# microsoft/MoGe

Measured on AMD Instinct MI355X. Metric: images/sec (MoGeModel.infer, moge-2-vitl 518x518 fp16), higher is better.
Workload: dtype f16

## Files before the change

moge_amd/csrc/attention_pp.hip:

```cpp
#include "common.h"

#define AP_GPTR(p) ((const __attribute__((address_space(1))) void*)(p))
#define AP_LPTR(p) ((__attribute__((address_space(3))) void*)(p))

typedef short s16x4 __attribute__((ext_vector_type(4)));

__device__ __forceinline__ u32x4 tr_pair(const char* p0, const char* p1) {
    const s16x4 a = __builtin_amdgcn_ds_read_tr16_b64_v4i16((__attribute__((address_space(3))) s16x4*)(p0));
    const s16x4 b = __builtin_amdgcn_ds_read_tr16_b64_v4i16((__attribute__((address_space(3))) s16x4*)(p1));
    typedef short s16x8 __attribute__((ext_vector_type(8)));
    const s16x8 v = {a[0], a[1], a[2], a[3], b[0], b[1], b[2], b[3]};
    return __builtin_bit_cast(u32x4, v);
}

__device__ __forceinline__ u32x4 pack8(const f32x16& p, int s) {
    f16x8 h;
#pragma unroll
    for (int i = 0; i < 8; i++) h[i] = (f16)p[8 * s + i];
    return __builtin_bit_cast(u32x4, h);
}

constexpr int AP_STAGE = 16384;
constexpr float AP_PSUM_LIMIT = 16384.f;

#ifdef MOGE_EXPERIMENTS
#include "../../tools/experiments/attention_pp_exp.inc"
#endif

constexpr int AP_VAR_DEFAULT = 0;
constexpr int AP_X_DEFAULT = 0;
constexpr int AP_KERN_DEFAULT = 3;
constexpr float AP_SCORE_LIMIT = 15.f;
constexpr float AP_ROWSUM_LIMIT = 49152.f;
template <int VAR>
__global__ __launch_bounds__(256, 3) void attn_pp16_kernel(const f16* __restrict__ q, const f16* __restrict__ k, const f16* __restrict__ v,
                                                           f16* __restrict__ out, int Ntok, int nh) {
    constexpr int NW = 4, NPW = 4;
    extern __shared__ __attribute__((aligned(16))) char smem[];

    const int tid = threadIdx.x, lane = tid & 63;
    const int wave = __builtin_amdgcn_readfirstlane(tid >> 6);
    const int l15 = lane & 15, g4 = lane >> 4;
    const int bh = blockIdx.y;
    const int b = bh / nh, head = bh - b * nh;
    const int q0 = blockIdx.x * (NW * 32) + wave * 32;

    u32x4 qf[2][2];
#pragma unroll
    for (int qb = 0; qb < 2; qb++) {
        const int qrow = q0 + qb * 16 + l15;
        const f16* qp = q + ((size_t)bh * Ntok + (qrow < Ntok ? qrow : Ntok - 1)) * 64;
#pragma unroll
        for (int ks = 0; ks < 2; ks++) qf[qb][ks] = *reinterpret_cast<const u32x4*>(qp + 32 * ks + 8 * g4);
    }

    const char* kbase = reinterpret_cast<const char*>(k + (size_t)bh * Ntok * 64);
    const char* vbase = reinterpret_cast<const char*>(v + (size_t)bh * Ntok * 64);
    const int prow = lane >> 3, pch = lane & 7;
    int drow[NPW];
    unsigned doff[NPW];
#pragma unroll
    for (int i = 0; i < NPW; i++) {
        const int p = wave + NW * i;
        const int row = (p & 7) * 8 + prow;
        drow[i] = row;
        const int ksw = ((row >> 1) & 1) | (((row >> 3) & 3) << 1);
        const int vsw = (((row >> 1) & 1) << 1) | (((row >> 3) & 1) << 2);
        doff[i] = (unsigned)(row * 128 + ((pch ^ (p >= 8 ? vsw : ksw)) << 4));
    }
    const int ntiles = (Ntok + 63) >> 6;
    auto issue = [&](int t) {
        char* st = smem + (t % 3) * AP_STAGE;
        const char* kt = uniform_ptr(kbase + (size_t)t * 8192);
        const char* vt = uniform_ptr(vbase + (size_t)t * 8192);
        if (t < ntiles - 1) {
#pragma unroll
            for (int i = 0; i < NPW; i++) {
                const int p = wave + NW * i;
                __builtin_amdgcn_global_load_lds(AP_GPTR((p >= 8 ? vt : kt) + doff[i]), AP_LPTR(st + p * 1024), 16, 0, 0);
            }
        } else {
#pragma unroll
            for (int i = 0; i < NPW; i++) {
                const int p = wave + NW * i;
                const int over = t * 64 + drow[i] - (Ntok - 1);
                const unsigned off = doff[i] - (over > 0 ? (unsigned)over * 128u : 0u);
                __builtin_amdgcn_global_load_lds(AP_GPTR((p >= 8 ? vt : kt) + off), AP_LPTR(st + p * 1024), 16, 0, 0);
            }
        }
    };

    const int kswl = ((l15 >> 1) & 1) | ((l15 >> 2) << 1);
    int kaddr[2];
#pragma unroll
    for (int ks = 0; ks < 2; ks++) kaddr[ks] = (8 * (l15 >> 2) + (l15 & 3)) * 128 + (((4 * ks + g4) ^ kswl) << 4);
    const int vswl = (((l15 >> 3) & 1) << 1) | ((g4 & 1) << 2);
    int vaddr[4];
#pragma unroll
    for (int db = 0; db < 4; db++)
        vaddr[db] = 8192 + (8 * g4 + (l15 >> 2)) * 128 + ((((2 * db) ^ vswl) | ((l15 & 3) >> 1)) << 4) + (l15 & 1) * 8;

    f32x4 o[4][2];
    f32x4 negs[2];
    float m_run[2], l_run[2];
#pragma unroll
    for (int qb = 0; qb < 2; qb++) {
#pragma unroll
        for (int db = 0; db < 4; db++) o[db][qb] = f32x4{0.f, 0.f, 0.f, 0.f};
        negs[qb] = f32x4{0.f, 0.f, 0.f, 0.f};
        m_run[qb] = -1e30f; l_run[qb] = 0.f;
    }

    issue(0);
    if (ntiles > 1) issue(1);

    int stage = 0;
    const char* ka[2];
    const char* va[4];
    f32x4 sc[4][2];
    float psum[2];
    auto tile_head = [&](int t) {
        if (t + 1 < ntiles) asm volatile("s_waitcnt vmcnt(%0)" ::"n"(NPW) : "memory");
        else asm volatile("s_waitcnt vmcnt(0)" ::: "memory");
        __builtin_amdgcn_s_barrier();
        asm volatile("" ::: "memory");
        if (t + 2 < ntiles) issue(t + 2);
        const int so = stage * AP_STAGE;
        stage = stage == 2 ? 0 : stage + 1;
#pragma unroll
        for (int ks = 0; ks < 2; ks++) ka[ks] = smem + (kaddr[ks] + so);
#pragma unroll
        for (int db = 0; db < 4; db++) va[db] = smem + (vaddr[db] + so);
    };
    auto pv = [&]() {
#pragma unroll
        for (int qb = 0; qb < 2; qb++) l_run[qb] += psum[qb];
#pragma unroll
        for (int s2 = 0; s2 < 2; s2++) {
            u32x4 pf[2];
#pragma unroll
            for (int qb = 0; qb < 2; qb++) {
                f16x8 hp;
#pragma unroll
                for (int r = 0; r < 4; r++) { hp[r] = (f16)sc[2 * s2][qb][r]; hp[4 + r] = (f16)sc[2 * s2 + 1][qb][r]; }
                pf[qb] = __builtin_bit_cast(u32x4, hp);
            }
#pragma unroll
            for (int db = 0; db < 4; db++) {
                const u32x4 vf = tr_pair(va[db] + (32 * ((VAR & 32) ? 0 : s2)) * 128, va[db] + (32 * ((VAR & 32) ? 0 : s2) + 4) * 128);
#pragma unroll
                for (int qb = 0; qb < 2; qb++) mma16<f16>(o[db][qb], vf, pf[qb]);
            }
        }
    };
    auto exact_body = [&](int t, bool last) {
#pragma unroll
        for (int kb = 0; kb < 4; kb++) {
            const int koff = (32 * (kb >> 1) + 4 * (kb & 1)) * 128;
            const u32x4 kf0 = *reinterpret_cast<const u32x4*>(ka[0] + koff), kf1 = *reinterpret_cast<const u32x4*>(ka[1] + koff);
#pragma unroll
            for (int qb = 0; qb < 2; qb++) {
                sc[kb][qb] = f32x4{0.f, 0.f, 0.f, 0.f};
                mma16<f16>(sc[kb][qb], kf0, qf[qb][0]);
                mma16<f16>(sc[kb][qb], kf1, qf[qb][1]);
            }
        }
#pragma unroll
        for (int qb = 0; qb < 2; qb++) {
            if (last) {
#pragma unroll
                for (int kb = 0; kb < 4; kb++)
#pragma unroll
                    for (int r = 0; r < 4; r++) {
                        const int key = t * 64 + 32 * (kb >> 1) + 8 * g4 + 4 * (kb & 1) + r;
                        if (key >= Ntok) sc[kb][qb][r] = -1e30f;
                    }
            }
            float mx = sc[0][qb][0];
#pragma unroll
            for (int kb = 0; kb < 4; kb++)
#pragma unroll
                for (int r = 0; r < 4; r++) mx = fmaxf(mx, sc[kb][qb][r]);
            mx = fmaxf(mx, __shfl_xor(mx, 16));
            mx = fmaxf(mx, __shfl_xor(mx, 32));
            const float m_new = fmaxf(m_run[qb], mx);
            const float alpha = __builtin_amdgcn_exp2f(m_run[qb] - m_new);
            m_run[qb] = m_new;
            l_run[qb] *= alpha;
#pragma unroll
            for (int db = 0; db < 4; db++)
#pragma unroll
                for (int r = 0; r < 4; r++) o[db][qb][r] *= alpha;
#pragma unroll
            for (int r = 0; r < 4; r++) negs[qb][r] = -m_new;
            float ps = 0.f;
#pragma unroll
            for (int kb = 0; kb < 4; kb++)
#pragma unroll
                for (int r = 0; r < 4; r++) {
                    sc[kb][qb][r] = __builtin_amdgcn_exp2f(sc[kb][qb][r] - m_new);
                    ps += sc[kb][qb][r];
                }
            psum[qb] = ps;
        }
        pv();
    };

    tile_head(0);
    exact_body(0, ntiles == 1);
    int t = 1;
    for (;;) {
        bool hit = false;
        for (; t < ntiles - 1; t++) {
            tile_head(t);
            if constexpr (VAR & 4) {
                u32x4 kf[4][2];
#pragma unroll
                for (int kb = 0; kb < 4; kb++) {
                    const int koff = (32 * (kb >> 1) + 4 * (kb & 1)) * 128;
                    kf[kb][0] = *reinterpret_cast<const u32x4*>(ka[0] + koff);
                    kf[kb][1] = *reinterpret_cast<const u32x4*>(ka[1] + koff);
                }
#pragma unroll
                for (int kb = 0; kb < 4; kb++)
#pragma unroll
                    for (int qb = 0; qb < 2; qb++)
                        sc[kb][qb] = __builtin_amdgcn_mfma_f32_16x16x32_f16(__builtin_bit_cast(f16x8, kf[kb][0]), __builtin_bit_cast(f16x8, qf[qb][0]), negs[qb], 0, 0, 0);
#pragma unroll
                for (int kb = 0; kb < 4; kb++)
#pragma unroll
                    for (int qb = 0; qb < 2; qb++) mma16<f16>(sc[kb][qb], kf[kb][1], qf[qb][1]);
            } else {
#pragma unroll
            for (int kb = 0; kb < 4; kb++) {
                const int koff = (32 * (kb >> 1) + 4 * (kb & 1)) * 128;
                const u32x4 kf0 = *reinterpret_cast<const u32x4*>(ka[0] + koff), kf1 = *reinterpret_cast<const u32x4*>(ka[1] + koff);
#pragma unroll
                for (int qb = 0; qb < 2; qb++) {
                    sc[kb][qb] = __builtin_amdgcn_mfma_f32_16x16x32_f16(__builtin_bit_cast(f16x8, kf0), __builtin_bit_cast(f16x8, qf[qb][0]), negs[qb], 0, 0, 0);
                    mma16<f16>(sc[kb][qb], kf1, qf[qb][1]);
                }
            }
            }
            bool trig = false;
            if constexpr ((VAR & 8) != 0) {
                float mx = sc[0][0][0];
#pragma unroll
                for (int kb = 0; kb < 4; kb++)
#pragma unroll
                    for (int qb = 0; qb < 2; qb++)
#pragma unroll
                        for (int r = 0; r < 4; r++) mx = fmaxf(mx, sc[kb][qb][r]);
                trig = !(mx <= AP_SCORE_LIMIT);
                if (__builtin_expect(__any(trig), 0)) { hit = true; break; }
            }
#pragma unroll
            for (int qb = 0; qb < 2; qb++) {
                float ps0 = 0.f, ps1 = 0.f;
#pragma unroll
                for (int kb = 0; kb < 4; kb++)
#pragma unroll
                    for (int r = 0; r < 4; r++) {
                        sc[kb][qb][r] = (VAR & 1) ? sc[kb][qb][r] * 1e-3f : __builtin_amdgcn_exp2f(sc[kb][qb][r]);
                        if (!(VAR & 16) || (kb == 0 && r == 0)) { if (kb & 1) ps1 += sc[kb][qb][r]; else ps0 += sc[kb][qb][r]; }
                    }
                psum[qb] = ps0 + ps1;
                trig |= !(psum[qb] < AP_PSUM_LIMIT);
            }
            if constexpr ((VAR & (2 | 8)) == 0) {
                if (__builtin_expect(__any(trig), 0)) { hit = true; break; }
            }
            pv();
        }
        if (!hit) break;
        exact_body(t, false);
        t++;
    }
    if (ntiles > 1) {
        tile_head(ntiles - 1);
        exact_body(ntiles - 1, true);
    }
#pragma unroll
    for (int qb = 0; qb < 2; qb++) {
        float l_tot = l_run[qb] + __shfl_xor(l_run[qb], 16);
        l_tot += __shfl_xor(l_tot, 32);
        const float inv = 1.f / l_tot;
        const int qrow = q0 + qb * 16 + l15;
        if (qrow < Ntok) {
            f16* op = out + ((size_t)b * Ntok + qrow) * ((size_t)nh * 64) + head * 64;
#pragma unroll
            for (int db = 0; db < 4; db++)
                store4(op + 16 * db + 4 * g4, o[db][qb][0] * inv, o[db][qb][1] * inv, o[db][qb][2] * inv, o[db][qb][3] * inv);
        }
    }
}

template <int QB> struct AttnAcc { f32x4 o[4][QB]; float m[QB], l[QB]; };
template <int QB, bool SK = false>
__device__ __forceinline__ bool attn_pp16mq_body(const f16* __restrict__ q, const f16* __restrict__ k, const f16* __restrict__ v, f16* __restrict__ out,
                                                 int Ntok, int nh, int bh, int q_base, char* smem, int tb_in = 0, int te_in = 0, AttnAcc<QB>* acc = nullptr,
                                                 const char* seed_k = nullptr) {
    constexpr int NW = 4, NPW = 4;
    const int tid = threadIdx.x, lane = tid & 63;
    const int wave = __builtin_amdgcn_readfirstlane(tid >> 6) & (NW - 1);
    const int l15 = lane & 15, g4 = lane >> 4;
    const int b = bh / nh, head = bh - b * nh;
    const int q0 = q_base + wave * (16 * QB);
    u32x4 qf[QB][2];
#pragma unroll
    for (int qb = 0; qb < QB; qb++) {
        const int qrow = q0 + qb * 16 + l15;
        const f16* qp = q + ((size_t)bh * Ntok + (qrow < Ntok ? qrow : Ntok - 1)) * 64;
#pragma unroll
        for (int ks = 0; ks < 2; ks++) qf[qb][ks] = *reinterpret_cast<const u32x4*>(qp + 32 * ks + 8 * g4);
    }
    const char* kbase = reinterpret_cast<const char*>(k + (size_t)bh * Ntok * 64);
    const char* vbase = reinterpret_cast<const char*>(v + (size_t)bh * Ntok * 64);
    const int prow = lane >> 3, pch = lane & 7;
    unsigned doff[NPW], doff_last[NPW];
    const int ntiles = (Ntok + 63) >> 6;
    const int tb = SK ? tb_in : 0, te = SK ? te_in : ntiles;
#pragma unroll
    for (int i = 0; i < NPW; i++) {
        const int p = wave + NW * i;
        const int row = (p & 7) * 8 + prow;
        const int ksw = ((row >> 1) & 1) | (((row >> 3) & 3) << 1);
        const int vsw = (((row >> 1) & 1) << 1) | (((row >> 3) & 1) << 2);
        doff[i] = (unsigned)(row * 128 + ((pch ^ (p >= 8 ? vsw : ksw)) << 4));
        const int over = (ntiles - 1) * 64 + row - (Ntok - 1);
        doff_last[i] = doff[i] - (over > 0 ? (unsigned)over * 128u : 0u);
    }
    auto issue = [&](int t) {
        char* st = smem + ((SK ? t - tb : t) % 3) * AP_STAGE;
        const char* kt = uniform_ptr(kbase + (size_t)t * 8192);
        const char* vt = uniform_ptr(vbase + (size_t)t * 8192);
        const bool last = t >= ntiles - 1;
#pragma unroll
        for (int i = 0; i < NPW; i++) {
            const int p = wave + NW * i;
            __builtin_amdgcn_global_load_lds(AP_GPTR((p >= 8 ? vt : kt) + (last ? doff_last[i] : doff[i])), AP_LPTR(st + p * 1024), 16, 0, 0);
        }
    };
    const int kswl = ((l15 >> 1) & 1) | ((l15 >> 2) << 1);
    int kaddr[2];
#pragma unroll
    for (int ks = 0; ks < 2; ks++) kaddr[ks] = (8 * (l15 >> 2) + (l15 & 3)) * 128 + (((4 * ks + g4) ^ kswl) << 4);
    const int vswl = (((l15 >> 3) & 1) << 1) | ((g4 & 1) << 2);
    int vaddr[4];
#pragma unroll
    for (int db = 0; db < 4; db++)
        vaddr[db] = 8192 + (8 * g4 + (l15 >> 2)) * 128 + ((((2 * db) ^ vswl) | ((l15 & 3) >> 1)) << 4) + (l15 & 1) * 8;

    f32x4 o[4][QB];
    f32x4 negs[QB];
    float m_run[QB], l_run[QB];
#pragma unroll
    for (int qb = 0; qb < QB; qb++) {
#pragma unroll
        for (int db = 0; db < 4; db++) o[db][qb] = f32x4{0.f, 0.f, 0.f, 0.f};
        negs[qb] = f32x4{0.f, 0.f, 0.f, 0.f};
        m_run[qb] = -1e30f; l_run[qb] = 0.f;
    }
    issue(tb);
    if (te - tb > 1) issue(tb + 1);

    int stage = 0;
    const char* ka[2];
    const char* va[4];
    f32x4 sc[4][QB];
    float psum[QB];
    auto tile_head = [&](int t, bool with_issue = true) {
        if (t + 1 < te) asm volatile("s_waitcnt vmcnt(%0)" ::"n"(NPW) : "memory");
        else asm volatile("s_waitcnt vmcnt(0)" ::: "memory");
        __builtin_amdgcn_s_barrier();
        asm volatile("" ::: "memory");
        if (with_issue && t + 2 < te) issue(t + 2);
        const int so = stage * AP_STAGE;
        stage = stage == 2 ? 0 : stage + 1;
#pragma unroll
        for (int ks = 0; ks < 2; ks++) ka[ks] = smem + (kaddr[ks] + so);
#pragma unroll
        for (int db = 0; db < 4; db++) va[db] = smem + (vaddr[db] + so);
    };
    auto pack = [&](int qb, u32x4 (&pf)[2]) {
#pragma unroll
        for (int s2 = 0; s2 < 2; s2++) {
            f16x8 hp;
#pragma unroll
            for (int r = 0; r < 4; r++) { hp[r] = (f16)sc[2 * s2][qb][r]; hp[4 + r] = (f16)sc[2 * s2 + 1][qb][r]; }
            pf[s2] = __builtin_bit_cast(u32x4, hp);
        }
    };
    auto pv_block = [&](int qb, const u32x4 (&pf)[2]) {
        l_run[qb] += psum[qb];
#pragma unroll
        for (int s2 = 0; s2 < 2; s2++)
#pragma unroll
            for (int db = 0; db < 4; db++) {
                const u32x4 vf = tr_pair(va[db] + (32 * s2) * 128, va[db] + (32 * s2 + 4) * 128);
                mma16<f16>(o[db][qb], vf, pf[s2]);
            }
    };
    auto exact_block = [&](int t, bool last, int qb) {
#pragma unroll
        for (int kb = 0; kb < 4; kb++) {
            const int koff = (32 * (kb >> 1) + 4 * (kb & 1)) * 128;
            const u32x4 kf0 = *reinterpret_cast<const u32x4*>(ka[0] + koff), kf1 = *reinterpret_cast<const u32x4*>(ka[1] + koff);
            sc[kb][qb] = f32x4{0.f, 0.f, 0.f, 0.f};
            mma16<f16>(sc[kb][qb], kf0, qf[qb][0]);
            mma16<f16>(sc[kb][qb], kf1, qf[qb][1]);
        }
        if (last) {
#pragma unroll
            for (int kb = 0; kb < 4; kb++)
#pragma unroll
                for (int r = 0; r < 4; r++) {
                    const int key = t * 64 + 32 * (kb >> 1) + 8 * g4 + 4 * (kb & 1) + r;
                    if (key >= Ntok) sc[kb][qb][r] = -1e30f;
                }
        }
        float mx = sc[0][qb][0];
#pragma unroll
        for (int kb = 0; kb < 4; kb++)
#pragma unroll
            for (int r = 0; r < 4; r++) mx = fmaxf(mx, sc[kb][qb][r]);
        mx = fmaxf(mx, __shfl_xor(mx, 16));
        mx = fmaxf(mx, __shfl_xor(mx, 32));
        const float m_new = fmaxf(m_run[qb], mx);
        const float alpha = __builtin_amdgcn_exp2f(m_run[qb] - m_new);
        m_run[qb] = m_new;
        l_run[qb] *= alpha;
#pragma unroll
        for (int db = 0; db < 4; db++)
#pragma unroll
            for (int r = 0; r < 4; r++) o[db][qb][r] *= alpha;
#pragma unroll
        for (int r = 0; r < 4; r++) negs[qb][r] = -m_new;
        float ps = 0.f;
#pragma unroll
        for (int kb = 0; kb < 4; kb++)
#pragma unroll
            for (int r = 0; r < 4; r++) {
                sc[kb][qb][r] = __builtin_amdgcn_exp2f(sc[kb][qb][r] - m_new);
                ps += sc[kb][qb][r];
            }
        ps += __shfl_xor(ps, 16);
        ps += __shfl_xor(ps, 32);
        psum[qb] = ps;
        u32x4 pf[2];
        pack(qb, pf);
        pv_block(qb, pf);
    };
    auto qk_block = [&](int qb, const u32x4 (&kf)[4][2]) {
#pragma unroll
        for (int kb = 0; kb < 4; kb++)
            sc[kb][qb] = __builtin_amdgcn_mfma_f32_16x16x32_f16(__builtin_bit_cast(f16x8, kf[kb][0]), __builtin_bit_cast(f16x8, qf[qb][0]), negs[qb], 0, 0, 0);
#pragma unroll
        for (int kb = 0; kb < 4; kb++) mma16<f16>(sc[kb][qb], kf[kb][1], qf[qb][1]);
    };
    u32x4 ones;
#pragma unroll
    for (int i = 0; i < 4; i++) ones[i] = 0x3c003c00u;
    const f32x4 zero4 = {0.f, 0.f, 0.f, 0.f};

    if (__builtin_amdgcn_readfirstlane(q0) >= Ntok) {
        for (int tt = tb; tt < te; tt++) tile_head(tt);
        return false;
    }
    bool seeded = false;
    if constexpr (SK) seeded = seed_k != nullptr && tb < ntiles - 1;
    tile_head(tb, !seeded);
    if constexpr (SK) if (seed_k) {
#pragma unroll
        for (int qb = 0; qb < QB; qb++) {
            float mx = -1e30f;
#pragma unroll
            for (int kb = 0; kb < 4; kb++) {
                const int koff = (32 * (kb >> 1) + 4 * (kb & 1)) * 128;
                const u32x4 kf0 = *reinterpret_cast<const u32x4*>(seed_k + kaddr[0] + koff), kf1 = *reinterpret_cast<const u32x4*>(seed_k + kaddr[1] + koff);
                f32x4 s0 = {0.f, 0.f, 0.f, 0.f};
                mma16<f16>(s0, kf0, qf[qb][0]);
                mma16<f16>(s0, kf1, qf[qb][1]);
#pragma unroll
                for (int r = 0; r < 4; r++) mx = fmaxf(mx, s0[r]);
            }
            mx = fmaxf(mx, __shfl_xor(mx, 16));
            mx = fmaxf(mx, __shfl_xor(mx, 32));
            m_run[qb] = mx;
#pragma unroll
            for (int r = 0; r < 4; r++) negs[qb][r] = -mx;
        }
    }
    int t = tb + 1;
    if (seeded) t = tb;
    else {
#pragma unroll
        for (int qb = 0; qb < QB; qb++) exact_block(tb, tb == ntiles - 1, qb);
    }
    const int hot_end = SK ? (te < ntiles - 1 ? te : ntiles - 1) : ntiles - 1;
    u32x4 pf[QB][2];
    f32x4 lt[QB];
    for (;;) {
        bool hit = false;
        for (; t < hot_end; t++) {
            if (!(seeded && t == tb)) tile_head(t, false);
            u32x4 kf[4][2];
#pragma unroll
            for (int kb = 0; kb < 4; kb++) {
                const int koff = (32 * (kb >> 1) + 4 * (kb & 1)) * 128;
                kf[kb][0] = *reinterpret_cast<const u32x4*>(ka[0] + koff);
                kf[kb][1] = *reinterpret_cast<const u32x4*>(ka[1] + koff);
            }
            __builtin_amdgcn_sched_barrier(0);
            if (t + 2 < te) issue(t + 2);
            __builtin_amdgcn_sched_barrier(0);
#pragma unroll
            for (int qb = 0; qb < QB; qb++) qk_block(qb, kf);
#pragma unroll
            for (int qb = 0; qb < QB; qb++) {
#pragma unroll
                for (int kb = 0; kb < 4; kb++)
#pragma unroll
                    for (int r = 0; r < 4; r++) sc[kb][qb][r] = __builtin_amdgcn_exp2f(sc[kb][qb][r]);
                pack(qb, pf[qb]);
                lt[qb] = __builtin_amdgcn_mfma_f32_16x16x32_f16(__builtin_bit_cast(f16x8, ones), __builtin_bit_cast(f16x8, pf[qb][0]), zero4, 0, 0, 0);
                mma16<f16>(lt[qb], ones, pf[qb][1]);
            }
            bool trig = false;
#pragma unroll
            for (int qb = 0; qb < QB; qb++) trig |= !(lt[qb][0] < AP_ROWSUM_LIMIT);
            if (__builtin_expect(__any(trig), 0)) { hit = true; break; }
#pragma unroll
            for (int qb = 0; qb < QB; qb++) l_run[qb] += lt[qb][0];
            {
                constexpr int AHEAD = QB == 4 ? 5 : 4;
                u32x4 vf[8];
                auto ld = [&](int gi) { vf[gi] = tr_pair(va[gi & 3] + (32 * (gi >> 2)) * 128, va[gi & 3] + (32 * (gi >> 2) + 4) * 128); };
#pragma unroll
                for (int gi = 0; gi < AHEAD; gi++) ld(gi);
                __builtin_amdgcn_sched_barrier(0);
#pragma unroll
                for (int gi = 0; gi < 8; gi++) {
                    if (gi + AHEAD < 8) ld(gi + AHEAD);
#pragma unroll
                    for (int qb = 0; qb < QB; qb++) mma16<f16>(o[gi & 3][qb], vf[gi], pf[qb][gi >> 2]);
                    __builtin_amdgcn_sched_barrier(0);
                }
            }
        }
        if (!hit) break;
#pragma unroll
        for (int qb = 0; qb < QB; qb++) {
            if (__any(!(lt[qb][0] < AP_ROWSUM_LIMIT))) exact_block(t, false, qb);
            else { psum[qb] = lt[qb][0]; pv_block(qb, pf[qb]); }
        }
        t++;
    }
    if (SK ? (te == ntiles && ntiles - 1 > tb) : (ntiles > 1)) {
        tile_head(ntiles - 1);
#pragma unroll
        for (int qb = 0; qb < QB; qb++) exact_block(ntiles - 1, true, qb);
    }
    if constexpr (SK) {
#pragma unroll
        for (int qb = 0; qb < QB; qb++) {
#pragma unroll
            for (int db = 0; db < 4; db++) acc->o[db][qb] = o[db][qb];
            acc->m[qb] = m_run[qb]; acc->l[qb] = l_run[qb];
        }
        return true;
    }
#pragma unroll
    for (int qb = 0; qb < QB; qb++) {
        const float inv = 1.f / l_run[qb];
        const int qrow = q0 + qb * 16 + l15;
        if (qrow < Ntok) {
            f16* op = out + ((size_t)b * Ntok + qrow) * ((size_t)nh * 64) + head * 64;
#pragma unroll
            for (int db = 0; db < 4; db++)
                store4(op + 16 * db + 4 * g4, o[db][qb][0] * inv, o[db][qb][1] * inv, o[db][qb][2] * inv, o[db][qb][3] * inv);
        }
    }
    return true;
}

template <int QB>
__global__ __launch_bounds__(256, QB > 2 ? 2 : 3) void attn_pp16mq_kernel(const f16* __restrict__ q, const f16* __restrict__ k, const f16* __restrict__ v,
                                                            f16* __restrict__ out, int Ntok, int nh, int xcd_remap, int q_start) {
    extern __shared__ __attribute__((aligned(16))) char smem[];
    int bh = blockIdx.y, qblk = blockIdx.x;
    if (((gridDim.y & 7) == 0) && (xcd_remap & 1)) {
        const int lin = blockIdx.y * gridDim.x + blockIdx.x;
        const int x = lin & 7, s = lin >> 3;
        const int hs = s / (int)gridDim.x;
        bh = x + 8 * hs;
        qblk = s - hs * (int)gridDim.x;
    }
    const int q_base = q_start + qblk * (64 * QB);
    if constexpr (QB == 4) if (xcd_remap & 2) {
        if (Ntok - q_base <= 128) { attn_pp16mq_body<2>(q, k, v, out, Ntok, nh, bh, q_base, smem); return; }
    }
    attn_pp16mq_body<QB>(q, k, v, out, Ntok, nh, bh, q_base, smem);
}

constexpr int AP_KS_MIN_TILES = 8;
template <int QB>
__global__ __launch_bounds__(512, 1) void attn_pp16ks_kernel(const f16* __restrict__ q, const f16* __restrict__ k, const f16* __restrict__ v,
                                                            f16* __restrict__ out, int Ntok, int nh, int xcd_remap, int tmid) {
    extern __shared__ __attribute__((aligned(16))) char smem[];
    int bh = blockIdx.y, qblk = blockIdx.x;
    if (((gridDim.y & 7) == 0) && (xcd_remap & 1)) {
        const int lin = blockIdx.y * gridDim.x + blockIdx.x;
        const int x = lin & 7, s = lin >> 3;
        const int hs = s / (int)gridDim.x;
        bh = x + 8 * hs;
        qblk = s - hs * (int)gridDim.x;
    }
    const int q_base = qblk * (64 * QB);
    const int tid = threadIdx.x, lane = tid & 63, t4 = tid & 255;
    const int wave8 = __builtin_amdgcn_readfirstlane(tid >> 6), grp = wave8 >> 2, wave = wave8 & 3;
    const int ntiles = (Ntok + 63) >> 6;
    AttnAcc<QB> a;
    const bool active = attn_pp16mq_body<QB, true>(q, k, v, out, Ntok, nh, bh, q_base, smem + grp * (3 * AP_STAGE), grp ? tmid : 0, grp ? ntiles : tmid, &a, grp ? smem : nullptr);
    for (int i = grp ? ntiles - tmid : tmid, n = max(tmid, ntiles - tmid); i < n; i++) __builtin_amdgcn_s_barrier();
    __syncthreads();
    f32x4* ex_o = reinterpret_cast<f32x4*>(smem);
    f32x2* ex_ml = reinterpret_cast<f32x2*>(smem + (size_t)4 * QB * 256 * 16);
    if (grp && active) {
#pragma unroll
        for (int db = 0; db < 4; db++)
#pragma unroll
            for (int qb = 0; qb < QB; qb++) ex_o[(db * QB + qb) * 256 + t4] = a.o[db][qb];
#pragma unroll
        for (int qb = 0; qb < QB; qb++) ex_ml[qb * 256 + t4] = f32x2{a.m[qb], a.l[qb]};
    }
    __syncthreads();
    if (grp || !active) return;
    const int l15 = lane & 15, g4 = lane >> 4;
    const int b = bh / nh, head = bh - b * nh;
    const int q0 = q_base + wave * (16 * QB);
#pragma unroll
    for (int qb = 0; qb < QB; qb++) {
        const f32x2 ml = ex_ml[qb * 256 + t4];
        const float mstar = fmaxf(a.m[qb], ml[0]);
        const float w0 = __builtin_amdgcn_exp2f(a.m[qb] - mstar), w1 = __builtin_amdgcn_exp2f(ml[0] - mstar);
        const float l = fmaf(w1, ml[1], w0 * a.l[qb]);
        const float inv = 1.f / l;
        const int qrow = q0 + qb * 16 + l15;
#pragma unroll
        for (int db = 0; db < 4; db++) {
            const f32x4 o1 = ex_o[(db * QB + qb) * 256 + t4];
            f32x4 o;
#pragma unroll
            for (int r = 0; r < 4; r++) o[r] = fmaf(w1, o1[r], w0 * a.o[db][qb][r]);
            if (qrow < Ntok) {
                f16* op = out + ((size_t)b * Ntok + qrow) * ((size_t)nh * 64) + head * 64;
                store4(op + 16 * db + 4 * g4, o[0] * inv, o[1] * inv, o[2] * inv, o[3] * inv);
            }
        }
    }
}

#ifdef MOGE_EXPERIMENTS
#include "../../tools/experiments/attention_pp16sk_exp.inc"
#else
size_t attention_pp_ws_bytes(int, int, int) { return 0; }
size_t attention_pp_ws_counter_bytes(int, int, int) { return 0; }
#endif

#ifdef MOGE_EXPERIMENTS
#include "../../tools/experiments/attention_pp16s_exp.inc"
#include "../../tools/experiments/attention_pp16x_exp.inc"
#endif


static int launch_attn_pp16(const void* q, const void* k, const void* v, void* out, int B, int nh, int Ntok, hipStream_t st, void* ws, size_t ws_bytes) {
    constexpr int smem = 3 * AP_STAGE;
#ifdef MOGE_EXPERIMENTS
    {
        int QB, nx, gx;
        if (ws && attn_sk_plan(B, nh, Ntok, &QB, &nx, &gx) && ws_bytes >= attention_pp_ws_bytes(B, nh, Ntok)) {
            int* cnt = reinterpret_cast<int*>(ws);
            float* part = reinterpret_cast<float*>(reinterpret_cast<char*>(ws) + attention_pp_ws_counter_bytes(B, nh, Ntok));
            if (QB == 4) {
                if (int rc = set_dyn_lds<attn_pp16sk_kernel<4>>(smem)) return rc;
                hipLaunchKernelGGL(attn_pp16sk_kernel<4>, dim3(nx * gx), dim3(256), smem, st, (const f16*)q, (const f16*)k, (const f16*)v, (f16*)out, Ntok, nh, nx, B * nh / nx, part, cnt);
            } else {
                if (int rc = set_dyn_lds<attn_pp16sk_kernel<2>>(smem)) return rc;
                hipLaunchKernelGGL(attn_pp16sk_kernel<2>, dim3(nx * gx), dim3(256), smem, st, (const f16*)q, (const f16*)k, (const f16*)v, (f16*)out, Ntok, nh, nx, B * nh / nx, part, cnt);
            }
            return (int)hipGetLastError();
        }
    }
#else
    (void)ws; (void)ws_bytes;
#endif
    dim3 grid((Ntok + 127) / 128, B * nh);
    const int akern = moge_tune_get("ATTN_KERN", AP_KERN_DEFAULT);
    if (akern >= 1) {
        const long wgs2 = (long)((Ntok + 127) / 128) * B * nh;
        const bool q4 = akern == 2 || akern == 4 || (akern == 3 && wgs2 > moge_tune_get("ATTN_Q2_MAX_WGS", 3 * pp_device_cus()));
        const int xr = (moge_tune_get("ATTN_XCD", 1) ? 1 : 0) | (moge_tune_get("ATTN_TAIL2", 1) ? 2 : 0);
#ifdef MOGE_EXPERIMENTS
        const int nfull = Ntok / 512, rem = Ntok - nfull * 512;
        const int nblk = nfull + (rem > 256 ? 1 : 0);
        const bool xk = nblk > 0 && (akern == 4 || (akern == 3 && moge_tune_get("ATTN_X", AP_X_DEFAULT) &&
                                                    (long)nblk * B * nh >= (long)moge_tune_get("ATTN_X_MIN_ROUNDS", 2) * pp_device_cus()));
        if (xk) {
            constexpr int smem_x = 4 * AP_STAGE + 8 * 8192;
            if (moge_tune_get("ATTN_X_TS", 0)) {
                static unsigned long long* dts = nullptr;
                if (!dts && hipMalloc(&dts, 16 * sizeof(unsigned long long)) != hipSuccess) return -1;
                (void)hipMemsetAsync(dts, 0, 16 * sizeof(unsigned long long), st);
                if (int rc = set_dyn_lds<attn_pp16x_kernel<0, 1>>(smem_x)) return rc;
                hipLaunchKernelGGL((attn_pp16x_kernel<0, 1>), dim3(nblk, B * nh), dim3(512), smem_x, st, (const f16*)q, (const f16*)k, (const f16*)v, (f16*)out, Ntok, nh, xr, dts);
                unsigned long long h[16];
                (void)hipMemcpyAsync(h, dts, sizeof(h), hipMemcpyDeviceToHost, st);
                (void)hipStreamSynchronize(st);
                for (int g2 = 0; g2 < 2; g2++)
                    if (h[g2 * 8 + 4])
                        fprintf(stderr, "[attn_pp16x ts] group %d: %llu hot tiles; per tile (s_memtime ticks): E body %.0f, barrier wait %.0f, M body %.0f, barrier wait %.0f\n", g2, h[g2 * 8 + 4],
                                (double)h[g2 * 8 + 0] / h[g2 * 8 + 4], (double)h[g2 * 8 + 1] / h[g2 * 8 + 4], (double)h[g2 * 8 + 2] / h[g2 * 8 + 4], (double)h[g2 * 8 + 3] / h[g2 * 8 + 4]);
            } else if (moge_tune_get("ATTN_X_PRIO", 0)) {
                if (int rc = set_dyn_lds<attn_pp16x_kernel<1>>(smem_x)) return rc;
                hipLaunchKernelGGL(attn_pp16x_kernel<1>, dim3(nblk, B * nh), dim3(512), smem_x, st, (const f16*)q, (const f16*)k, (const f16*)v, (f16*)out, Ntok, nh, xr);
            } else {
                if (int rc = set_dyn_lds<attn_pp16x_kernel<0>>(smem_x)) return rc;
                hipLaunchKernelGGL(attn_pp16x_kernel<0>, dim3(nblk, B * nh), dim3(512), smem_x, st, (const f16*)q, (const f16*)k, (const f16*)v, (f16*)out, Ntok, nh, xr);
            }
            const int covered = nblk * 512;
            if (covered < Ntok) {
                if (int rc = set_dyn_lds<attn_pp16mq_kernel<4>>(smem)) return rc;
                hipLaunchKernelGGL(attn_pp16mq_kernel<4>, dim3((Ntok - covered + 255) / 256, B * nh), dim3(256), smem, st, (const f16*)q, (const f16*)k, (const f16*)v, (f16*)out, Ntok, nh, xr, covered);
            }
            return (int)hipGetLastError();
        }
#endif
#ifdef MOGE_EXPERIMENTS
        const int sfull = Ntok / 256;
        if ((akern == 6 || akern == 7) && sfull > 0 && Ntok > 128) {
            constexpr int smem_s = APS_NSTG * AP_STAGE + 4 * 8192;
            if (akern == 6) {
                if (int rc = set_dyn_lds<attn_pp16s_kernel<1>>(smem_s)) return rc;
                hipLaunchKernelGGL(attn_pp16s_kernel<1>, dim3(sfull, B * nh), dim3(256), smem_s, st, (const f16*)q, (const f16*)k, (const f16*)v, (f16*)out, Ntok, nh, xr);
            } else {
                constexpr int smem_s2 = 5 * AP_STAGE;
                if (int rc = set_dyn_lds<attn_pp16s_kernel<2>>(smem_s2)) return rc;
                hipLaunchKernelGGL(attn_pp16s_kernel<2>, dim3(sfull, B * nh), dim3(256), smem_s2, st, (const f16*)q, (const f16*)k, (const f16*)v, (f16*)out, Ntok, nh, xr);
            }
            const int covered = sfull * 256;
            if (covered < Ntok) {
                if (int rc = set_dyn_lds<attn_pp16mq_kernel<4>>(smem)) return rc;
                hipLaunchKernelGGL(attn_pp16mq_kernel<4>, dim3((Ntok - covered + 255) / 256, B * nh), dim3(256), smem, st, (const f16*)q, (const f16*)k, (const f16*)v, (f16*)out, Ntok, nh, xr, covered);
            }
            return (int)hipGetLastError();
        }
#endif
        if (const int ks = moge_tune_get("ATTN_KS", 1); ks > 1 || (ks == 1 && akern == 3)) {
            constexpr int smem_ks = 6 * AP_STAGE;
            const int cus = pp_device_cus(), ntiles = (Ntok + 63) >> 6;
            const long w2 = (long)((Ntok + 127) / 128) * B * nh, w4 = (long)((Ntok + 255) / 256) * B * nh;
            const bool fits = ks == 1 && ntiles >= AP_KS_MIN_TILES;
            int tmid = (ntiles + 1) >> 1;
            if (const int f = moge_tune_get("ATTN_KS_MID", 0); f > 0 && f < ntiles) tmid = f;
            if ((ks == 2 && ntiles >= 2) || (fits && w2 <= cus)) {
                if (int rc = set_dyn_lds<attn_pp16ks_kernel<2>>(smem_ks)) return rc;
                hipLaunchKernelGGL(attn_pp16ks_kernel<2>, dim3((Ntok + 127) / 128, B * nh), dim3(512), smem_ks, st, (const f16*)q, (const f16*)k, (const f16*)v, (f16*)out, Ntok, nh, xr, tmid);
                return (int)hipGetLastError();
            }
            if ((ks == 4 && ntiles >= 2) || (fits && w4 <= cus)) {
                if (int rc = set_dyn_lds<attn_pp16ks_kernel<4>>(smem_ks)) return rc;
                hipLaunchKernelGGL(attn_pp16ks_kernel<4>, dim3((Ntok + 255) / 256, B * nh), dim3(512), smem_ks, st, (const f16*)q, (const f16*)k, (const f16*)v, (f16*)out, Ntok, nh, xr, tmid);
                return (int)hipGetLastError();
            }
        }
        if (q4) {
            if (int rc = set_dyn_lds<attn_pp16mq_kernel<4>>(smem)) return rc;
            hipLaunchKernelGGL(attn_pp16mq_kernel<4>, dim3((Ntok + 255) / 256, B * nh), dim3(256), smem, st, (const f16*)q, (const f16*)k, (const f16*)v, (f16*)out, Ntok, nh, xr, 0);
        } else {
            if (int rc = set_dyn_lds<attn_pp16mq_kernel<2>>(smem)) return rc;
            hipLaunchKernelGGL(attn_pp16mq_kernel<2>, grid, dim3(256), smem, st, (const f16*)q, (const f16*)k, (const f16*)v, (f16*)out, Ntok, nh, xr, 0);
        }
        return (int)hipGetLastError();
    }
#define AP_LAUNCH_VAR(V) do { if (int rc = set_dyn_lds<attn_pp16_kernel<V>>(smem)) return rc; \
        hipLaunchKernelGGL(attn_pp16_kernel<V>, grid, dim3(256), smem, st, (const f16*)q, (const f16*)k, (const f16*)v, (f16*)out, Ntok, nh); \
        return (int)hipGetLastError(); } while (0)
#ifdef MOGE_EXPERIMENTS
    switch (moge_tune_get("ATTN_VAR", AP_VAR_DEFAULT)) {
    case 0: AP_LAUNCH_VAR(0);
    case 1: AP_LAUNCH_VAR(1);
    case 2: AP_LAUNCH_VAR(2);
    case 4: AP_LAUNCH_VAR(4);
    case 6: AP_LAUNCH_VAR(6);
    case 8: AP_LAUNCH_VAR(8);
    case 12: AP_LAUNCH_VAR(12);
    case 16: AP_LAUNCH_VAR(16);
    case 18: AP_LAUNCH_VAR(18);
    case 19: AP_LAUNCH_VAR(19);
    case 32: AP_LAUNCH_VAR(32);
    case 50: AP_LAUNCH_VAR(50);
    case 51: AP_LAUNCH_VAR(51);
    default: return -1;
    }
#else
    AP_LAUNCH_VAR(AP_VAR_DEFAULT);
#endif
#undef AP_LAUNCH_VAR
}

#ifdef MOGE_EXPERIMENTS
template <int NW, int QT>
static int launch_attn_pp_cfg(const void* q, const void* k, const void* v, void* out, int B, int nh, int Ntok, hipStream_t st) {
    constexpr int smem = 3 * AP_STAGE;
    constexpr auto kern = attn_pp_kernel<NW, QT>;
    if (int rc = set_dyn_lds<kern>(smem)) return rc;
    dim3 grid((Ntok + NW * 32 * QT - 1) / (NW * 32 * QT), B * nh);
    hipLaunchKernelGGL(kern, grid, dim3(NW * 64), smem, st, (const f16*)q, (const f16*)k, (const f16*)v, (f16*)out, Ntok, nh);
    return (int)hipGetLastError();
}
#endif

int launch_attention_pp(const void* q, const void* k, const void* v, void* out, int B, int nh, int Ntok, hipStream_t st, void* ws, size_t ws_bytes) {
    if (Ntok < 1) return -1;
#ifdef MOGE_EXPERIMENTS
    switch (moge_tune_get("ATTN_EXP", 0)) {
    case 1: return launch_attn_pp_cfg<4, 1>(q, k, v, out, B, nh, Ntok, st);
    case 2: return launch_attn_pp_cfg<4, 2>(q, k, v, out, B, nh, Ntok, st);
    case 3: return launch_attn_pp_cfg<8, 1>(q, k, v, out, B, nh, Ntok, st);
    default: break;
    }
#endif
    return launch_attn_pp16(q, k, v, out, B, nh, Ntok, st, ws, ws_bytes);
}
```

Baseline: 237.4.

## Pack two heads' tail query blocks into one workgroup for attention

```diff
diff --git a/moge_amd/csrc/attention_pp.hip b/moge_amd/csrc/attention_pp.hip
--- a/moge_amd/csrc/attention_pp.hip
+++ b/moge_amd/csrc/attention_pp.hip
@@ -1,4 +1,7 @@
 #include "common.h"
+
+#include <cstdio>
+#include <vector>
 
 #define AP_GPTR(p) ((const __attribute__((address_space(1))) void*)(p))
 #define AP_LPTR(p) ((__attribute__((address_space(3))) void*)(p))
@@ -30,6 +33,7 @@
 constexpr int AP_VAR_DEFAULT = 0;
 constexpr int AP_X_DEFAULT = 0;
 constexpr int AP_KERN_DEFAULT = 3;
+constexpr int AP_TAILPACK_DEFAULT = 2;
 constexpr float AP_SCORE_LIMIT = 15.f;
 constexpr float AP_ROWSUM_LIMIT = 49152.f;
 template <int VAR>
@@ -296,11 +300,13 @@
 }
 
 template <int QB> struct AttnAcc { f32x4 o[4][QB]; float m[QB], l[QB]; };
-template <int QB, bool SK = false>
+template <int QB, bool SK = false, int NW = 4, int NSTG = 3>
 __device__ __forceinline__ bool attn_pp16mq_body(const f16* __restrict__ q, const f16* __restrict__ k, const f16* __restrict__ v, f16* __restrict__ out,
                                                  int Ntok, int nh, int bh, int q_base, char* smem, int tb_in = 0, int te_in = 0, AttnAcc<QB>* acc = nullptr,
                                                  const char* seed_k = nullptr) {
-    constexpr int NW = 4, NPW = 4;
+    static_assert(NW == 2 || NW == 4, "a ring's 16 one-KiB pieces per tile are split evenly over its waves");
+    static_assert(NSTG == 2 || NSTG == 3, "ring depth");
+    constexpr int NPW = 16 / NW, DIST = NSTG - 1;
     const int tid = threadIdx.x, lane = tid & 63;
     const int wave = __builtin_amdgcn_readfirstlane(tid >> 6) & (NW - 1);
     const int l15 = lane & 15, g4 = lane >> 4;
@@ -317,7 +323,8 @@
     const char* kbase = reinterpret_cast<const char*>(k + (size_t)bh * Ntok * 64);
     const char* vbase = reinterpret_cast<const char*>(v + (size_t)bh * Ntok * 64);
     const int prow = lane >> 3, pch = lane & 7;
-    unsigned doff[NPW], doff_last[NPW];
+    constexpr int NOFF = NW == 2 ? NPW / 2 : NPW;
+    unsigned doff[NOFF], doff_last[NOFF];
     const int ntiles = (Ntok + 63) >> 6;
     const int tb = SK ? tb_in : 0, te = SK ? te_in : ntiles;
 #pragma unroll
@@ -326,19 +333,22 @@
         const int row = (p & 7) * 8 + prow;
         const int ksw = ((row >> 1) & 1) | (((row >> 3) & 3) << 1);
         const int vsw = (((row >> 1) & 1) << 1) | (((row >> 3) & 1) << 2);
-        doff[i] = (unsigned)(row * 128 + ((pch ^ (p >= 8 ? vsw : ksw)) << 4));
+        const unsigned d = (unsigned)(row * 128 + ((pch ^ (p >= 8 ? vsw : ksw)) << 4));
         const int over = (ntiles - 1) * 64 + row - (Ntok - 1);
-        doff_last[i] = doff[i] - (over > 0 ? (unsigned)over * 128u : 0u);
+        const unsigned dl = d - (over > 0 ? (unsigned)over * 128u : 0u);
+        if (i < NOFF) { doff[i] = d; doff_last[i] = dl; }
+        else { doff[i - NOFF] |= d << 16; doff_last[i - NOFF] |= dl << 16; }
     }
     auto issue = [&](int t) {
-        char* st = smem + ((SK ? t - tb : t) % 3) * AP_STAGE;
+        char* st = smem + ((SK ? t - tb : t) % NSTG) * AP_STAGE;
         const char* kt = uniform_ptr(kbase + (size_t)t * 8192);
         const char* vt = uniform_ptr(vbase + (size_t)t * 8192);
         const bool last = t >= ntiles - 1;
 #pragma unroll
         for (int i = 0; i < NPW; i++) {
             const int p = wave + NW * i;
-            __builtin_amdgcn_global_load_lds(AP_GPTR((p >= 8 ? vt : kt) + (last ? doff_last[i] : doff[i])), AP_LPTR(st + p * 1024), 16, 0, 0);
+            const unsigned o = last ? doff_last[i % NOFF] : doff[i % NOFF];
+            __builtin_amdgcn_global_load_lds(AP_GPTR((p >= 8 ? vt : kt) + (NOFF == NPW ? o : i < NOFF ? o & 0xffffu : o >> 16)), AP_LPTR(st + p * 1024), 16, 0, 0);
         }
     };
     const int kswl = ((l15 >> 1) & 1) | ((l15 >> 2) << 1);
@@ -362,7 +372,7 @@
         m_run[qb] = -1e30f; l_run[qb] = 0.f;
     }
     issue(tb);
-    if (te - tb > 1) issue(tb + 1);
+    if (DIST > 1 && te - tb > 1) issue(tb + 1);
 
     int stage = 0;
     const char* ka[2];
@@ -370,13 +380,13 @@
     f32x4 sc[4][QB];
     float psum[QB];
     auto tile_head = [&](int t, bool with_issue = true) {
-        if (t + 1 < te) asm volatile("s_waitcnt vmcnt(%0)" ::"n"(NPW) : "memory");
+        if (DIST > 1 && t + 1 < te) asm volatile("s_waitcnt vmcnt(%0)" ::"n"(NPW) : "memory");
         else asm volatile("s_waitcnt vmcnt(0)" ::: "memory");
         __builtin_amdgcn_s_barrier();
         asm volatile("" ::: "memory");
-        if (with_issue && t + 2 < te) issue(t + 2);
+        if (with_issue && t + DIST < te) issue(t + DIST);
         const int so = stage * AP_STAGE;
-        stage = stage == 2 ? 0 : stage + 1;
+        stage = stage == NSTG - 1 ? 0 : stage + 1;
 #pragma unroll
         for (int ks = 0; ks < 2; ks++) ka[ks] = smem + (kaddr[ks] + so);
 #pragma unroll
@@ -391,19 +401,22 @@
             pf[s2] = __builtin_bit_cast(u32x4, hp);
         }
     };
-    auto pv_block = [&](int qb, const u32x4 (&pf)[2]) {
+    auto pv_block = [&](int qb, const u32x4 (&pf)[2], bool lo_only = false) {
         l_run[qb] += psum[qb];
 #pragma unroll
         for (int s2 = 0; s2 < 2; s2++)
 #pragma unroll
             for (int db = 0; db < 4; db++) {
+                if (s2 == 1 && lo_only) break;
                 const u32x4 vf = tr_pair(va[db] + (32 * s2) * 128, va[db] + (32 * s2 + 4) * 128);
                 mma16<f16>(o[db][qb], vf, pf[s2]);
             }
     };
     auto exact_block = [&](int t, bool last, int qb) {
+        const bool lo_only = last && t * 64 + 32 >= Ntok;
 #pragma unroll
         for (int kb = 0; kb < 4; kb++) {
+            if (kb >= 2 && lo_only) { sc[kb][qb] = f32x4{-1e30f, -1e30f, -1e30f, -1e30f}; continue; }
             const int koff = (32 * (kb >> 1) + 4 * (kb & 1)) * 128;
             const u32x4 kf0 = *reinterpret_cast<const u32x4*>(ka[0] + koff), kf1 = *reinterpret_cast<const u32x4*>(ka[1] + koff);
             sc[kb][qb] = f32x4{0.f, 0.f, 0.f, 0.f};
@@ -441,6 +454,7 @@
         for (int kb = 0; kb < 4; kb++)
 #pragma unroll
             for (int r = 0; r < 4; r++) {
+                if (kb >= 2 && lo_only) { sc[kb][qb][r] = 0.f; continue; }
                 sc[kb][qb][r] = __builtin_amdgcn_exp2f(sc[kb][qb][r] - m_new);
                 ps += sc[kb][qb][r];
             }
@@ -449,7 +463,7 @@
         psum[qb] = ps;
         u32x4 pf[2];
         pack(qb, pf);
-        pv_block(qb, pf);
+        pv_block(qb, pf, lo_only);
     };
     auto qk_block = [&](int qb, const u32x4 (&kf)[4][2]) {
 #pragma unroll
@@ -512,7 +526,7 @@
                 kf[kb][1] = *reinterpret_cast<const u32x4*>(ka[1] + koff);
             }
             __builtin_amdgcn_sched_barrier(0);
-            if (t + 2 < te) issue(t + 2);
+            if (t + DIST < te) issue(t + DIST);
             __builtin_amdgcn_sched_barrier(0);
 #pragma unroll
             for (int qb = 0; qb < QB; qb++) qk_block(qb, kf);
@@ -585,9 +599,43 @@
 }
 
 template <int QB>
-__global__ __launch_bounds__(256, QB > 2 ? 2 : 3) void attn_pp16mq_kernel(const f16* __restrict__ q, const f16* __restrict__ k, const f16* __restrict__ v,
-                                                            f16* __restrict__ out, int Ntok, int nh, int xcd_remap, int q_start) {
-    extern __shared__ __attribute__((aligned(16))) char smem[];
+__device__ __forceinline__ int attn_pp16mq_wg(const f16* __restrict__ q, const f16* __restrict__ k, const f16* __restrict__ v, f16* __restrict__ out,
+                                              int Ntok, int nh, int xcd_remap, int q_start, int nbh, char* smem) {
+    if constexpr (QB == 4) if (xcd_remap & 4) {
+        const int nfull = Ntok >> 8, nfw = nfull * nbh, ntw = (nbh + 1) >> 1;
+        const bool first = (xcd_remap & 8) != 0, remap = (xcd_remap & 1) && (nbh & 15) == 0;
+        const int lin = blockIdx.x;
+        const bool tail = first ? lin < ntw : lin >= nfw;
+        if (!tail) {
+            const int f = first ? lin - ntw : lin;
+            int bh, qblk;
+            if (remap) {
+                const int x = f & 7, s = f >> 3, hs = s / nfull;
+                bh = x + 8 * hs;
+                qblk = s - hs * nfull;
+            } else {
+                bh = f / nfull;
+                qblk = f - bh * nfull;
+            }
+            attn_pp16mq_body<4>(q, k, v, out, Ntok, nh, bh, qblk * 256, smem);
+            return 0;
+        }
+        const int j = first ? lin : lin - nfw;
+        const int pair = __builtin_amdgcn_readfirstlane(threadIdx.x >> 6) >> 1;
+        const int bh = remap ? (j & 7) + 8 * (2 * (j >> 3) + pair) : 2 * j + pair;
+        const int q_base = nfull * 256, rest = Ntok - q_base;
+        char* ring = smem + pair * (2 * AP_STAGE);
+        if (bh >= nbh) {
+            for (int t = 0, nt = (Ntok + 63) >> 6; t < nt; t++) __builtin_amdgcn_s_barrier();
+        } else if (rest <= 32) {
+            attn_pp16mq_body<1, false, 2, 2>(q, k, v, out, Ntok, nh, bh, q_base, ring);
+        } else if (rest <= 64) {
+            attn_pp16mq_body<2, false, 2, 2>(q, k, v, out, Ntok, nh, bh, q_base, ring);
+        } else {
+            attn_pp16mq_body<4, false, 2, 2>(q, k, v, out, Ntok, nh, bh, q_base, ring);
+        }
+        return 2;
+    }
     int bh = blockIdx.y, qblk = blockIdx.x;
     if (((gridDim.y & 7) == 0) && (xcd_remap & 1)) {
         const int lin = blockIdx.y * gridDim.x + blockIdx.x;
@@ -598,9 +646,30 @@
     }
     const int q_base = q_start + qblk * (64 * QB);
     if constexpr (QB == 4) if (xcd_remap & 2) {
-        if (Ntok - q_base <= 128) { attn_pp16mq_body<2>(q, k, v, out, Ntok, nh, bh, q_base, smem); return; }
+        if (Ntok - q_base <= 128) { attn_pp16mq_body<2>(q, k, v, out, Ntok, nh, bh, q_base, smem); return 1; }
     }
     attn_pp16mq_body<QB>(q, k, v, out, Ntok, nh, bh, q_base, smem);
+    return 0;
+}
+
+template <int QB>
+__global__ __launch_bounds__(256, QB > 2 ? 2 : 3) void attn_pp16mq_kernel(const f16* __restrict__ q, const f16* __restrict__ k, const f16* __restrict__ v,
+                                                            f16* __restrict__ out, int Ntok, int nh, int xcd_remap, int q_start, int nbh,
+                                                            unsigned long long* ts) {
+    extern __shared__ __attribute__((aligned(16))) char smem[];
+    unsigned long long* wts = nullptr;
+    if (ts) {
+        wts = ts + 4 * (size_t)(blockIdx.y * gridDim.x + blockIdx.x);
+        if (threadIdx.x == 0) {
+            wts[0] = __builtin_amdgcn_s_memtime();
+            wts[2] = (unsigned)__builtin_amdgcn_s_getreg((31 << 11) | 4) | ((unsigned long long)(unsigned)__builtin_amdgcn_s_getreg((31 << 11) | 20) << 32);
+        }
+    }
+    const int kind = attn_pp16mq_wg<QB>(q, k, v, out, Ntok, nh, xcd_remap, q_start, nbh, smem);
+    if (wts && (threadIdx.x & 63) == 0) {
+        atomicMax(wts + 1, (unsigned long long)__builtin_amdgcn_s_memtime());
+        if (threadIdx.x == 0) wts[3] = (unsigned long long)kind;
+    }
 }
 
 constexpr int AP_KS_MIN_TILES = 8;
@@ -676,6 +745,7 @@
 
 static int launch_attn_pp16(const void* q, const void* k, const void* v, void* out, int B, int nh, int Ntok, hipStream_t st, void* ws, size_t ws_bytes) {
     constexpr int smem = 3 * AP_STAGE;
+    constexpr int smem_q4 = 4 * AP_STAGE;
 #ifdef MOGE_EXPERIMENTS
     {
         int QB, nx, gx;
@@ -730,8 +800,8 @@
             }
             const int covered = nblk * 512;
             if (covered < Ntok) {
-                if (int rc = set_dyn_lds<attn_pp16mq_kernel<4>>(smem)) return rc;
-                hipLaunchKernelGGL(attn_pp16mq_kernel<4>, dim3((Ntok - covered + 255) / 256, B * nh), dim3(256), smem, st, (const f16*)q, (const f16*)k, (const f16*)v, (f16*)out, Ntok, nh, xr, covered);
+                if (int rc = set_dyn_lds<attn_pp16mq_kernel<4>>(smem_q4)) return rc;
+                hipLaunchKernelGGL(attn_pp16mq_kernel<4>, dim3((Ntok - covered + 255) / 256, B * nh), dim3(256), smem, st, (const f16*)q, (const f16*)k, (const f16*)v, (f16*)out, Ntok, nh, xr, covered, B * nh, nullptr);
             }
             return (int)hipGetLastError();
         }
@@ -750,8 +820,8 @@
             }
             const int covered = sfull * 256;
             if (covered < Ntok) {
-                if (int rc = set_dyn_lds<attn_pp16mq_kernel<4>>(smem)) return rc;
-                hipLaunchKernelGGL(attn_pp16mq_kernel<4>, dim3((Ntok - covered + 255) / 256, B * nh), dim3(256), smem, st, (const f16*)q, (const f16*)k, (const f16*)v, (f16*)out, Ntok, nh, xr, covered);
+                if (int rc = set_dyn_lds<attn_pp16mq_kernel<4>>(smem_q4)) return rc;
+                hipLaunchKernelGGL(attn_pp16mq_kernel<4>, dim3((Ntok - covered + 255) / 256, B * nh), dim3(256), smem, st, (const f16*)q, (const f16*)k, (const f16*)v, (f16*)out, Ntok, nh, xr, covered, B * nh, nullptr);
             }
             return (int)hipGetLastError();
         }
@@ -775,11 +845,31 @@
             }
         }
         if (q4) {
-            if (int rc = set_dyn_lds<attn_pp16mq_kernel<4>>(smem)) return rc;
-            hipLaunchKernelGGL(attn_pp16mq_kernel<4>, dim3((Ntok + 255) / 256, B * nh), dim3(256), smem, st, (const f16*)q, (const f16*)k, (const f16*)v, (f16*)out, Ntok, nh, xr, 0);
+            const int rest = Ntok & 255, nbh = B * nh;
+            const bool pack = rest >= 1 && rest <= 128 && moge_tune_get("ATTN_TAILPACK", AP_TAILPACK_DEFAULT) == 2;
+            const int xq = xr | (pack ? 4 : 0) | (pack && moge_tune_get("ATTN_TAIL_FIRST", 1) ? 8 : 0);
+            const dim3 g4 = pack ? dim3((Ntok >> 8) * nbh + ((nbh + 1) >> 1)) : dim3((Ntok + 255) / 256, nbh);
+            const int lds = pack ? smem_q4 : smem;
+            if (int rc = set_dyn_lds<attn_pp16mq_kernel<4>>(smem_q4)) return rc;
+            if (moge_tune_get("ATTN_WG_TS", 0)) {
+                const size_t nwg = (size_t)g4.x * g4.y;
+                unsigned long long* dts = nullptr;
+                if (hipMalloc(&dts, nwg * 32) != hipSuccess) return -1;
+                (void)hipMemsetAsync(dts, 0, nwg * 32, st);
+                hipLaunchKernelGGL(attn_pp16mq_kernel<4>, g4, dim3(256), lds, st, (const f16*)q, (const f16*)k, (const f16*)v, (f16*)out, Ntok, nh, xq, 0, nbh, dts);
+                std::vector<unsigned long long> h(nwg * 4);
+                (void)hipMemcpyAsync(h.data(), dts, nwg * 32, hipMemcpyDeviceToHost, st);
+                (void)hipStreamSynchronize(st);
+                (void)hipFree(dts);
+                fprintf(stderr, "[attn wg ts] B %d nh %d N %d tailpack %d tail_first %d wgs %zu: wg,t_start,t_end,hw_id,xcc_id,kind\n", B, nh, Ntok, pack ? 2 : 0, (xq & 8) ? 1 : 0, nwg);
+                for (size_t w = 0; w < nwg; w++)
+                    fprintf(stderr, "[attn wg ts] %zu,%llu,%llu,%llu,%llu,%llu\n", w, h[4 * w], h[4 * w + 1], h[4 * w + 2] & 0xffffffffull, h[4 * w + 2] >> 32, h[4 * w + 3]);
+            } else {
+                hipLaunchKernelGGL(attn_pp16mq_kernel<4>, g4, dim3(256), lds, st, (const f16*)q, (const f16*)k, (const f16*)v, (f16*)out, Ntok, nh, xq, 0, nbh, nullptr);
+            }
         } else {
             if (int rc = set_dyn_lds<attn_pp16mq_kernel<2>>(smem)) return rc;
-            hipLaunchKernelGGL(attn_pp16mq_kernel<2>, grid, dim3(256), smem, st, (const f16*)q, (const f16*)k, (const f16*)v, (f16*)out, Ntok, nh, xr, 0);
+            hipLaunchKernelGGL(attn_pp16mq_kernel<2>, grid, dim3(256), smem, st, (const f16*)q, (const f16*)k, (const f16*)v, (f16*)out, Ntok, nh, xr, 0, B * nh, nullptr);
         }
         return (int)hipGetLastError();
     }
```

Measured after the change: 237.9 (median of 6 runs). Within noise of the previous version (+0.2%).
